# xipengwang/AprilSAM

Hardware: NVIDIA H100
Metric: Gauss-Newton solves/sec (batch + incremental) on M3500 & 100k-pose graph (higher is better)
Workload: dtype f64

## Files before the change

aprilsam_b200/csrc/asam_cuda.cu:

```cuda

#include <cuda_runtime.h>

#include <climits>
#include <cmath>
#include <cstdarg>
#include <cstdint>
#include <cstdio>
#include <cstdlib>
#include <cstring>
#include <ctime>
#include <vector>

#include "asam_cuda.h"

#define ASAM_EXPORT extern "C" __attribute__((visibility("default")))

static thread_local char g_err[512] = "";

static int set_err(const char *fmt, ...)
{
    va_list ap;
    va_start(ap, fmt);
    vsnprintf(g_err, sizeof(g_err), fmt, ap);
    va_end(ap);
// ... 1526 lines not shown
    for (int rep = 0; rep < 4; rep++) {
        CK(cudaEventRecord(d->tev[0], d->stream));
        k_fp64_peak<<<d->n_sm, threads, 0, d->stream>>>((double *) d->partial.p, iters);
        CK(cudaGetLastError());
        CK(cudaEventRecord(d->tev[1], d->stream));
        CK(cudaEventSynchronize(d->tev[1]));
        float ms = 0.f;
        CK(cudaEventElapsedTime(&ms, d->tev[0], d->tev[1]));
        const double tf = 2.0 * 8 * iters * (double) threads * d->n_sm / (ms * 1e-3) * 1e-12;
        if (rep > 0 && tf > best)
            best = tf;
    }
    *tflops_out = best;
    return 0;
}

ASAM_EXPORT int asam_device_info(asam_dev_t *d, int *n_sm, int *fac_grid, int *fac_smem, int *bs_grid)
{
    *n_sm = d->n_sm;
    *fac_grid = d->fac_grid;
    *fac_smem = d->fac_smem;
    *bs_grid = d->bs_grid;
    return 0;
}

ASAM_EXPORT int asam_set_trace(asam_dev_t *d, int enabled)
{
    d->trace_on = enabled;
    return 0;
}

ASAM_EXPORT int asam_download_trace(asam_dev_t *d, int which, unsigned long long *out, int max_tasks)
{
    CK(cudaSetDevice(d->device));
    if (flush_uploads(d))
        return 1;
    int n = which == 0 ? d->trace_nfac : d->trace_nbs;
    Buf &b = which == 0 ? d->trace_fac : d->trace_bs;
    if (n > max_tasks)
        n = max_tasks;
    if (n <= 0 || !b.p)
        return 0;
    CK(cudaMemcpyAsync(out, b.p, (size_t) n * 8 * sizeof(unsigned long long), cudaMemcpyDeviceToHost, d->stream));
    CK(cudaStreamSynchronize(d->stream));
    return 0;
}

ASAM_EXPORT int asam_set_panel_trace(asam_dev_t *d, int sn, int max_panels)
{
    CK(cudaSetDevice(d->device));
    d->ptrace_sn = -1;
    if (sn < 0 || max_panels <= 0)
        return 0;
    const size_t bytes = (size_t) max_panels * 64 * sizeof(unsigned long long);
    if (buf_reserve(d, d->ptrace, bytes, false, false) || flush_uploads(d))
        return 1;
    CK(cudaMemsetAsync(d->ptrace.p, 0, bytes, d->stream));
    d->ptrace_sn = sn;
    d->ptrace_panels = max_panels;
    return 0;
}

ASAM_EXPORT int asam_download_panel_trace(asam_dev_t *d, unsigned long long *out, int max_panels)
{
    CK(cudaSetDevice(d->device));
    if (!d->ptrace.p || max_panels > d->ptrace_panels)
        return set_err("asam_download_panel_trace: no trace");
    if (flush_uploads(d))
        return 1;
    CK(cudaMemcpyAsync(out, d->ptrace.p, (size_t) max_panels * 64 * sizeof(unsigned long long), cudaMemcpyDeviceToHost, d->stream));
    CK(cudaStreamSynchronize(d->stream));
    return 0;
}

ASAM_EXPORT int asam_set_timing(asam_dev_t *d, int enabled)
{
    d->timing = enabled;
    d->ev_set[0] = d->ev_set[1] = d->ev_set[2] = 0;
    return 0;
}

ASAM_EXPORT int asam_last_kernel_ms(asam_dev_t *d, float *lin_ms, float *fac_ms, float *bs_ms)
{
    CK(cudaSetDevice(d->device));
    if (flush_uploads(d))
        return 1;
    CK(cudaStreamSynchronize(d->stream));
    float *outs[3] = { lin_ms, fac_ms, bs_ms };
    for (int i = 0; i < 3; i++) {
        float ms = 0.f;
        if (d->ev_set[i])
            CK(cudaEventElapsedTime(&ms, d->ev[2 * i], d->ev[2 * i + 1]));
        if (outs[i])
            *outs[i] = ms;
    }
    return 0;
}
```

aprilsam_b200/csrc/asam_kernels.cuh:

```cuda
#pragma once

#include <cuda_runtime.h>

#include <cstdint>

#include "asam_cuda.h"

#define ASAM_TR_FLAG (1 << 30)
#define ASAM_MAX_CACHED_CHILDREN 24

__device__ __forceinline__ double d_mod2pi(double v)
{
    const double twopi = 6.2831853071795862319959;
    const double pi = 3.141592653589793238462643383279502884196;
    double w = v + pi;
    return (w - twopi * floor(w / twopi)) - pi;
}

__device__ __forceinline__ void d_atb(const double *A, const double *B, double *C)
{
#pragma unroll
    for (int i = 0; i < 3; i++)
#pragma unroll
        for (int j = 0; j < 3; j++) {
// ... 26 lines not shown
        r[i] = A[i * 3 + 0] * v[0] + A[i * 3 + 1] * v[1] + A[i * 3 + 2] * v[2];
}

__device__ __forceinline__ void d_xyt_eval(const double *pa, const double *pb, const double *z, double *Ja,
                                           double *Jb, double *r)
{
    double ca, sa;
    sincos(pa[2], &sa, &ca);
    double dx = pb[0] - pa[0], dy = pb[1] - pa[1];
    double zh0 = ca * dx + sa * dy;
    double zh1 = -sa * dx + ca * dy;
    double zh2 = pb[2] - pa[2];
    Ja[0] = -ca; Ja[1] = -sa; Ja[2] = -sa * dx + ca * dy;
    Ja[3] = sa;  Ja[4] = -ca; Ja[5] = -ca * dx - sa * dy;
    Ja[6] = 0.0; Ja[7] = 0.0; Ja[8] = -1.0;
    Jb[0] = ca;  Jb[1] = sa;  Jb[2] = 0.0;
    Jb[3] = -sa; Jb[4] = ca;  Jb[5] = 0.0;
    Jb[6] = 0.0; Jb[7] = 0.0; Jb[8] = 1.0;
    r[0] = z[0] - zh0;
    r[1] = z[1] - zh1;
    r[2] = d_mod2pi(z[2] - zh2);
}

__device__ __forceinline__ bool d_two_pose(const int type) { return type == 1 || type == 32; }

__device__ __forceinline__ double d_loss_weight(const int loss, const double k, const double s)
{
    const double k2 = k * k;
    if (loss == 1)
        return s <= k2 ? 1.0 : k / sqrt(s);
    return 1.0 / (1.0 + s / k2);
}

__device__ __forceinline__ double d_loss_rho(const int loss, const double k, const double s)
{
    const double k2 = k * k;
    if (loss == 1)
        return s <= k2 ? s : 2.0 * k * sqrt(s) - k2;
    return k2 * log1p(s / k2);
}

__device__ __forceinline__ double d_rsqrt_in_range(const double a)
{
    double y = (double) rsqrtf((float) a);
    double e = fma(-a * y, y, 1.0);
    y = fma(0.5 * y, e, y);
    e = fma(-a * y, y, 1.0);
    y = fma(0.5 * y, e, y);
    return y;
}

__device__ __forceinline__ double d_rsqrt(const double a)
{
    if (!(a >= 0x1p-120 && a <= 0x1p120)) {
        if (!(a > 0.0 && a < INFINITY))
            return rsqrt(a);
        int ex;
        frexp(a, &ex);
        const int h = ex / 2;
        return ldexp(d_rsqrt_in_range(ldexp(a, -2 * h)), -h);
    }
    return d_rsqrt_in_range(a);
}

__device__ __forceinline__ int ld_volatile(const int *p) { return *((const volatile int *) p); }

__device__ __forceinline__ int ld_acquire(const int *p)
{
    int v;
    asm volatile("ld.acquire.gpu.global.b32 %0, [%1];" : "=r"(v) : "l"(p) : "memory");
    return v;
}
__device__ __forceinline__ void st_release(int *p, const int v)
{
    asm volatile("st.release.gpu.global.b32 [%0], %1;" ::"l"(p), "r"(v) : "memory");
}
__device__ __forceinline__ void red_release_add(int *p, const int v)
{
    asm volatile("red.release.gpu.global.add.s32 [%0], %1;" ::"l"(p), "r"(v) : "memory");
}

__device__ __forceinline__ unsigned long long d_now()
{
    unsigned long long t;
    asm volatile("mov.u64 %0, %%globaltimer;" : "=l"(t));
    return t;
}

struct SpinClock {
    long long n = 0;
    unsigned long long t0 = 0;
};
__device__ __forceinline__ bool spin_over(SpinClock &c, long long limit_ns)
{
    if ((++c.n & 1023) != 0)
        return false;
    const unsigned long long now = d_now();
    if (c.t0 == 0) {
        c.t0 = now;
        return false;
    }
    return (long long) (now - c.t0) > limit_ns;
}


struct LinArgs {
    const int *f_type, *f_a, *f_b, *f_slot;
    const double *f_z, *f_W;
    const double2 *f_loss;
    const double *lp, *st;
    const double *pts;
    const int *node2q;
    double *Adiag, *Aoff, *Bq;
    int f_first, f_count;
};
// ... 299 lines not shown
            const double x2 = (p2[i] - x0 * l20 - x1 * l21) * r2;
            p0[i] = x0;
            p1[i] = x1;
            p2[i] = x2;
        }
        PF_SYNC();
        if (tid == 0) {
            p0[rb] = a00 * r0; p0[rb + 1] = l10; p0[rb + 2] = l20;
            p1[rb + 1] = d1 * r1; p1[rb + 2] = l21;
            p2[rb + 2] = d2 * r2;
            if (dinv_out) {
                dinv_out[rb] = r0; dinv_out[rb + 1] = r1; dinv_out[rb + 2] = r2;
            }
        }
        const int nrem = pb - (c0 + 3);
        const int nrow = m - (rb + 3) + 1;
        if (nrem > 0 && nrow > 0) {
            int ng = g_pf_groups ? nt / nrow : 1;
            ng = ng > nrem ? nrem : ng;
            if (ng > 1) {
                const int gi = tid / nrow, ri = tid - gi * nrow;
                if (gi < ng) {
                    const int i = rb + 3 + ri;
                    const double x0 = p0[i], x1 = p1[i], x2 = p2[i];
                    const int jmax = min(nrem, ri + 1);
                    for (int jj = gi; jj < jmax; jj += ng) {
                        const int jr = rb + 3 + jj;
                        double *pj = P + (size_t) (c0 + 3 + jj) * ldp;
                        pj[i] -= x0 * p0[jr] + x1 * p1[jr] + x2 * p2[jr];
                    }
                }
            } else {
                for (int i = i_first; i <= m; i += nt) {
                    const double x0 = p0[i], x1 = p1[i], x2 = p2[i];
                    const int jmax = min(nrem, i - (rb + 3) + 1);
                    for (int jj = 0; jj < jmax; jj++) {
                        const int jr = rb + 3 + jj;
                        double *pj = P + (size_t) (c0 + 3 + jj) * ldp;
                        pj[i] -= x0 * p0[jr] + x1 * p1[jr] + x2 * p2[jr];
                    }
                }
            }
        }
    }
    PF_SYNC();
#undef PF_SYNC
}

#define ASAM_TPB 48
#define ASAM_TROWS 256
#define ASAM_TCOLS 64

#define ASAM_CROWS 128

__device__ __forceinline__ unsigned smem_u32(const void *p) { return (unsigned) __cvta_generic_to_shared(p); }

__device__ __forceinline__ void mbar_init(unsigned long long *bar, unsigned count)
{
    asm volatile("mbarrier.init.shared::cta.b64 [%0], %1;" ::"r"(smem_u32(bar)), "r"(count) : "memory");
    asm volatile("fence.mbarrier_init.release.cluster;" ::: "memory");
}

__device__ __forceinline__ void mbar_expect_tx(unsigned long long *bar, unsigned bytes)
{
    asm volatile("mbarrier.arrive.expect_tx.shared::cta.b64 _, [%0], %1;" ::"r"(smem_u32(bar)), "r"(bytes) : "memory");
}

__device__ __forceinline__ void mbar_wait(unsigned long long *bar, unsigned parity)
{
    unsigned ok;
    long long tries = 0;
    do {
        asm volatile("{\n\t.reg .pred p;\n\tmbarrier.try_wait.parity.shared::cta.b64 p, [%1], %2;\n\tselp.u32 %0, 1, 0, p;\n\t}"
                     : "=r"(ok)
                     : "r"(smem_u32(bar)), "r"(parity)
                     : "memory");
        if (!ok && ++tries > (1LL << 24))
            __trap();
    } while (!ok);
}

__device__ __forceinline__ void bulk_g2s(void *dst, const void *src, unsigned bytes, unsigned long long *bar)
{
    asm volatile("cp.async.bulk.shared::cluster.global.mbarrier::complete_tx::bytes [%0], [%1], %2, [%3];" ::"r"(smem_u32(dst)),
                 "l"(src), "r"(bytes), "r"(smem_u32(bar))
                 : "memory");
}

#define ASAM_LDW 52
#define ASAM_WS_DOUBLES(m) (2 * (size_t) ((m) + 2) * ASAM_LDW)

template <int MT>
__device__ __noinline__ void tile_rm(double *F, const int ld, const double *Wk, const int pb4, const int cb0, const int ncol,
                                     const int rb0, const int nrow, const int out_mode, double *Out, double *Li, double *Lj,
                                     unsigned long long *bar, unsigned &parity)
{
    const int tid = threadIdx.x;
    const int lane = tid & 31, warp = tid >> 5;
    const bool same = rb0 == cb0 && nrow >= ncol;
    __syncthreads();
    if (warp == 0) {
        asm volatile("fence.proxy.async;" ::: "memory");
        if (lane == 0) {
            const unsigned bi = (unsigned) nrow * ASAM_LDW * 8u, bj = same ? 0u : (unsigned) ncol * ASAM_LDW * 8u;
            mbar_expect_tx(bar, bi + bj);
            bulk_g2s(Li, Wk + (size_t) rb0 * ASAM_LDW, bi, bar);
// ... 56 lines not shown
                        else if (out_mode == 1)
                            Out[ii + jj * ASAM_TPB] = acc[mt][q][e];
                        else
                            Out[ii + jj * ASAM_TROWS] = acc[mt][q][e];
                    }
                }
    }
}

struct TeamCtx {
    int *tbar_s;
    int G, w, phase;
    long long spin_limit;
    int *err;
    int sn;
};

__device__ __forceinline__ bool team_barrier(TeamCtx &tc, int *s_flag)
{
    __syncthreads();
    if (threadIdx.x == 0) {
        red_release_add(tc.tbar_s, 1);
        const int target = (++tc.phase) * tc.G;
        SpinClock spins;
        int ok = 1;
        while (ld_volatile(tc.tbar_s) < target) {
            __nanosleep(20);
            if (spin_over(spins, tc.spin_limit) || ld_volatile(tc.err) < 0) {
                atomicCAS(tc.err, 0, -(1 + tc.sn));
                ok = 0;
                break;
            }
        }
        ld_acquire(tc.tbar_s);
        *s_flag = ok;
    } else {
        tc.phase++;
    }
    __syncthreads();
    return *s_flag != 0;
}

__device__ __forceinline__ void team_leave(TeamCtx &tc)
{
    if (threadIdx.x == 0) {
        const int v = atomicAdd(tc.tbar_s, 1);
        if (v == tc.phase * tc.G + tc.G - 1)
            atomicExch(tc.tbar_s, 0);
    }
}

__device__ __forceinline__ bool team_owns(int col, int w, int G) { return ((col >> 2) % G) == w; }

__device__ __forceinline__ void diag_factor_rl(double *D, int pb, double *rdv, int sn_id, int *err)
{
    constexpr int LDD = ASAM_TPB;
    constexpr int SUB = 256;
    if (threadIdx.x < SUB) {
        for (int k1 = 0; k1 < pb; k1 += ASAM_PB) {
            const int pbb = min(ASAM_PB, pb - k1);
            panel_factor(D + (size_t) k1 * LDD, LDD, k1, pbb, pb - 1, sn_id, err, rdv, SUB);
            if (k1 + pbb < pb) {
                trailing_update_mma(D, LDD, D + (size_t) k1 * LDD, LDD, pbb, k1 + pbb, pb, pb - 1, SUB / 32);
                bar_sub(SUB);
            }
        }
    }
    __syncthreads();
}

__device__ __forceinline__ void trsm_row_block(double *Li, const double *D, const double *rdv, const int b0, const int nb,
                                               double *Frow, int ld, double *Wrow)
{
    const int tid = threadIdx.x;
    constexpr int LDD = ASAM_TPB;
    double r[12];
#pragma unroll
    for (int q = 0; q < 12; q++)
        r[q] = (q < nb) ? Li[tid + (b0 + q) * ASAM_TROWS] : 0.0;
    for (int p = 0; p < b0; p++) {
        const double xp = Li[tid + p * ASAM_TROWS];
        const double2 *Dp = reinterpret_cast<const double2 *>(D + p * LDD + b0);
#pragma unroll
        for (int q2 = 0; q2 < 6; q2++) {
            const double2 v = Dp[q2];
            r[2 * q2] -= xp * v.x;
            r[2 * q2 + 1] -= xp * v.y;
        }
    }
#pragma unroll
    for (int q = 0; q < 12; q++) {
        if (q < nb) {
            r[q] *= rdv[b0 + q];
#pragma unroll
            for (int q2 = q + 1; q2 < 12; q2++)
                r[q2] -= r[q] * D[(b0 + q2) + (b0 + q) * LDD];
        }
    }
#pragma unroll
    for (int q = 0; q < 12; q++)
        if (q < nb) {
            Li[tid + (b0 + q) * ASAM_TROWS] = r[q];
            Frow[(size_t) (b0 + q) * ld] = r[q];
            Wrow[b0 + q] = r[q];
        }
}

__device__ __forceinline__ void trsm_row(double *Li, const double *D, const double *rdv, int pb, double *Frow, int ld,
                                         double *Wrow)
{
    for (int b0 = 0; b0 < pb; b0 += 12)
        trsm_row_block(Li, D, rdv, b0, min(12, pb - b0), Frow, ld, Wrow);
    for (int q = pb; q < ((pb + 3) & ~3); q++)
        Wrow[q] = 0.0;
// ... 106 lines not shown
    if (!team_barrier(tc, s_flag))
        return false;
    if (w == 0 && nw > 0 && tid == 0)
        a.arrive[s] = 0;
    unsigned long long t_panel = 0, t_mark = 0;
    if (trow && tid == 0)
        trow[3] = d_now();

    double *D = sm;
    double *rdv = D + ASAM_TPB * ASAM_TPB;
    double *Li = rdv + ASAM_TPB;
    double *Lj = Li + ASAM_TROWS * ASAM_LDW;
    double *Wbase = F + (size_t) ld * m;
    auto Wbuf = [&](int panel_index) { return Wbase + (size_t) (panel_index & 1) * (m + 2) * ASAM_LDW; };
    double *dinv = a.dinv + 3 * (size_t) d.first;
    int *crew_bar = a.tbar + 2 * (size_t) s + 1;

    auto tile = [&](int k0, int pb, int cb0, int ncol, int rb0, int nrow, double *Dout) {
        const double *Wk = Wbuf(k0 / ASAM_TPB);
        const int pb4 = (pb + 3) & ~3;
        if (Dout)
            tile_rm<1>(F, ld, Wk, pb4, cb0, ncol, rb0, nrow, 1, Dout, Li, Lj, mbar, mb_parity);
        else if (nrow <= 128)
            tile_rm<2>(F, ld, Wk, pb4, cb0, ncol, rb0, nrow, 0, nullptr, Li, Lj, mbar, mb_parity);
        else
            tile_rm<4>(F, ld, Wk, pb4, cb0, ncol, rb0, nrow, 0, nullptr, Li, Lj, mbar, mb_parity);
    };
    auto panel = [&](int k0, int pb, int rb0) {
        __syncthreads();
        for (int e = tid; e < ASAM_TPB * ASAM_TPB; e += nt) {
            const int i = e % ASAM_TPB, j = e / ASAM_TPB;
            D[e] = (i >= j && i < pb && j < pb) ? __ldcg(&F[(k0 + i) + (size_t) (k0 + j) * ld]) : 0.0;
        }
        const int i = rb0 + tid;
        const bool row = rb0 >= 0 && i >= k0 + pb && i <= m;
        if (row)
            for (int j = 0; j < pb; j++)
                Li[tid + j * ASAM_TROWS] = __ldcg(&F[i + (size_t) (k0 + j) * ld]);
        __syncthreads();
        diag_factor_rl(D, pb, rdv, s, err);
        if (row)
            trsm_row(Li, D, rdv, pb, F + i + (size_t) k0 * ld, ld, Wbuf(0) + (size_t) i * ASAM_LDW);
    };
    auto writeback = [&](int k0, int pb) {
        for (int e = tid; e < pb * pb; e += nt) {
            const int i = e % pb, j = e / pb;
            if (i >= j)
                F[(k0 + i) + (size_t) (k0 + j) * ld] = D[i + j * ASAM_TPB];
        }
        for (int e = tid; e < pb; e += nt)
            dinv[k0 + e] = rdv[e];
    };

    auto diag_publish = [&](int k0, int pb, int seq) {
        __syncthreads();
        constexpr int LDD = ASAM_TPB;
        constexpr int SUB = 256;
        int stage = 0;
        for (int k1 = 0; k1 < pb; k1 += ASAM_PB) {
            const int pbb = min(ASAM_PB, pb - k1);
            panel_factor(D + (size_t) k1 * LDD, LDD, k1, pbb, pb - 1, s, err, rdv, SUB);
            ++stage;
            for (int e = tid; e < pbb * pb; e += SUB) {
                const int j = k1 + e / pb, i = e % pb;
                if (i >= j)
                    F[(k0 + i) + (size_t) (k0 + j) * ld] = D[i + j * LDD];
            }
            for (int e = tid; e < pbb; e += SUB)
                dinv[k0 + k1 + e] = rdv[k1 + e];
            bar_sub(SUB);
            if (tid == 0)
                st_release(crew_bar, 8 * seq + stage);
            if (k1 + pbb < pb) {
                trailing_update_mma(D, LDD, D + (size_t) k1 * LDD, LDD, pbb, k1 + pbb, pb, pb - 1, SUB / 32);
                bar_sub(SUB);
            }
        }
        __syncthreads();
    };
    auto rows_solve_staged = [&](int k0, int pb, int rb0, int seq, double *Wnext) {
        constexpr int LDD = ASAM_TPB;
        if (tid == 0)
            *s_flag = 1;
        __syncthreads();
        const int i = rb0 + tid;
        const bool row = tid < ASAM_CROWS && i <= m;
        int stage = 0;
        for (int b0 = 0; b0 < pb; b0 += ASAM_PB, ++stage) {
            const int nb = min(ASAM_PB, pb - b0);
            if (warp >= 4) {
                if (tid == 128 && *s_flag) {
                    SpinClock spins;
                    while (ld_volatile(crew_bar) < 8 * seq + stage + 1) {
                        __nanosleep(20);
                        if (spin_over(spins, a.spin_limit) || ld_volatile(err) < 0) {
                            atomicCAS(err, 0, -(1 + s));
                            *s_flag = 0;
                            break;
                        }
                    }
                    ld_acquire(crew_bar);
                }
                asm volatile("bar.sync 2, 128;" ::: "memory");
                if (*s_flag) {
                    for (int e = tid - 128; e < nb * ASAM_TPB; e += 128) {
                        const int j = b0 + e / ASAM_TPB, ii = e % ASAM_TPB;
                        D[ii + j * LDD] = (ii >= j && ii < pb) ? __ldcg(&F[(k0 + ii) + (size_t) (k0 + j) * ld]) : 0.0;
                    }
                    if (tid - 128 < nb)
                        rdv[b0 + tid - 128] = __ldcg(&dinv[k0 + b0 + tid - 128]);
                }
                __threadfence_block();
                asm volatile("bar.arrive %0, 256;" ::"r"(3 + stage) : "memory");
            } else {
                asm volatile("bar.sync %0, 256;" ::"r"(3 + stage) : "memory");
                if (row && *s_flag)
                    trsm_row_block(Li, D, rdv, b0, nb, F + i + (size_t) k0 * ld, ld, Wnext + (size_t) i * ASAM_LDW);
            }
        }
        if (row && *s_flag)
            for (int q = pb; q < ((pb + 3) & ~3); q++)
                Wnext[(size_t) i * ASAM_LDW + q] = 0.0;
        __syncthreads();
        return *s_flag != 0;
    };
    {
        const int pb = min(ASAM_TPB, c);
        if (trow && tid == 0)
            t_mark = d_now();
        const int nchunk = (m + 1 + ASAM_TROWS - 1) / ASAM_TROWS;
        bool first = true;
        for (int ch = w; ch < nchunk || first; ch += G) {
            panel(0, pb, ch < nchunk ? ch * ASAM_TROWS : -1);
            first = false;
        }
        if (!team_barrier(tc, s_flag))
            return false;
        if (trow && tid == 0)
            t_panel += d_now() - t_mark;
        if (w == 0)
            writeback(0, pb);
    }
    int seq = 0;
    const bool pt_on = a.ptrace && s == a.ptrace_sn && w < 8 && tid == 0;
    for (int k0 = 0; k0 < c; k0 += ASAM_TPB) {
        unsigned long long *pt = (pt_on && k0 / ASAM_TPB < a.ptrace_panels) ? a.ptrace + ((size_t) (k0 / ASAM_TPB) * 8 + w) * 8 : nullptr;
        if (pt) {
            pt[0] = d_now();
            pt[1] = pt[2] = pt[3] = pt[0];
            pt[5] = (unsigned long long) m;
            pt[6] = (unsigned long long) G;
        }
        const int pb = min(ASAM_TPB, c - k0);
        const int kn0 = k0 + pb;
        const bool has_next = kn0 < c;
        const int pbn = has_next ? min(ASAM_TPB, c - kn0) : 0;
        const int ncrew = has_next ? 1 + (m - (kn0 + pbn) + 1 + ASAM_CROWS - 1) / ASAM_CROWS : 0;
        ++seq;
        if (w < ncrew) {
            if (trow && tid == 0)
                t_mark = d_now();
            if (w == 0) {
                __syncthreads();
                for (int e = tid; e < ASAM_TPB * ASAM_TPB; e += nt)
                    D[e] = 0.0;
                tile(k0, pb, kn0, pbn, kn0, pbn, D);
                if (pt)
                    pt[1] = d_now();
                diag_publish(kn0, pbn, seq);
                if (pt)
                    pt[2] = d_now();
            }
            for (int it = (w == 0 ? G : w); it < ncrew; it += G) {
                const int rb0 = kn0 + pbn + (it - 1) * ASAM_CROWS;
                tile_rm<2>(F, ld, Wbuf(k0 / ASAM_TPB), (pb + 3) & ~3, kn0, pbn, rb0, min(ASAM_CROWS, m - rb0 + 1), 2, Li, Li,
                           Lj, mbar, mb_parity);
                if (pt && w > 0 && it == w)
                    pt[1] = d_now();
                if (!rows_solve_staged(kn0, pbn, rb0, seq, Wbuf(kn0 / ASAM_TPB)))
                    return false;
            }
            if (pt && w > 0)
                pt[2] = d_now();
            if (trow && tid == 0)
                t_panel += d_now() - t_mark;
        }

        const int j0 = kn0 + pbn;
        const int nfree = (G - ncrew >= 2) ? G - ncrew : G, wfree = (G - ncrew >= 2) ? w - ncrew : w;
        int n256 = 0;
        for (int cb0 = j0; cb0 < m; cb0 += ASAM_TCOLS)
            n256 += (m - cb0 + 1 + 255) / 256;
        const int TR = (n256 < 2 * nfree) ? 128 : 256;
        if (wfree >= 0) {
            int u = 0;
            for (int cb0 = j0; cb0 < m; cb0 += ASAM_TCOLS)
                for (int rb0 = cb0; rb0 <= m; rb0 += TR, ++u)
                    if (u % nfree == wfree)
                        tile(k0, pb, cb0, min(ASAM_TCOLS, m - cb0), rb0, min(TR, m - rb0 + 1), nullptr);
        }
        if (pt)
            pt[3] = d_now();
        if (!team_barrier(tc, s_flag))
            return false;
        if (pt) {
            pt[4] = d_now();
            pt[7] = (unsigned long long) ncrew;
        }
    }
    if (w == 0 && tid == 0)
        atomicExch(crew_bar, 0);

    if (trow && tid == 0) {
        trow[4] = d_now();
        trow[7] = (unsigned long long) (unsigned) m | (t_panel << 32);
    }
    if (w == 0) {
        for (int e = tid; e < c; e += nt)
            a.y[3 * (size_t) d.first + e] = __ldcg(&F[m + (size_t) e * ld]);
        __syncthreads();
        if (tid == 0 && d.parent >= 0) {
            __threadfence();
            atomicAdd(&a.arrive[d.parent], 1);
        }
    }
    team_leave(tc);
    __syncthreads();
    return true;
}

__device__ __forceinline__ void ticket_release(int *ticket, int *done)
{
// ... 579 lines not shown
            __threadfence();
            atomicAdd(&a.arrive[d.parent], 1);
        }
        __syncwarp();
    }
    ticket_release(&a.ctrl[5], &a.ctrl[6]);
}

struct BsArgs {
    const asam_sn_desc_t *sn;
    const int *ipool;
    const double *arena;
    const double *y;
    const double *dinv;
    double *x;
    int *xdone;
    const int *btasks;
    const int *bfirst;
    int *xblk;
    int ntasks;
    int *ctrl;
    int epoch;
    int smem_doubles;
    long long spin_limit;
    unsigned long long *trace;
};

#define ASAM_BSW 96
#define ASAM_BT_SN(e) ((e) & 0xffffff)
#define ASAM_BT_BLK(e) ((((e) >> 24) & 0x7f) - 1)

template <int U>
__device__ __forceinline__ double bs_dot(const double *lk, const double *xs, int n, int lane)
{
    double acc0 = 0.0, acc1 = 0.0;
    for (int i0 = lane; i0 < n; i0 += 32 * U) {
        double v[U];
#pragma unroll
        for (int u = 0; u < U; u++)
            v[u] = (i0 + 32 * u < n) ? lk[i0 + 32 * u] : 0.0;
#pragma unroll
        for (int u = 0; u < U; u += 2) {
            acc0 += v[u] * xs[min(i0 + 32 * u, n - 1)];
            acc1 += v[u + 1] * xs[min(i0 + 32 * (u + 1), n - 1)];
        }
    }
    acc0 += acc1;
#pragma unroll
    for (int o = 16; o > 0; o >>= 1)
        acc0 += __shfl_down_sync(0xffffffffu, acc0, o);
    return acc0;
}

__device__ bool cta_backsolve(const BsArgs &a, const int t, const int s, double *sm, int *s_abort, const int jcol = 0,
                              const int blk_only = -1)
{
    const int tid = threadIdx.x, nt = blockDim.x;
    const int lane = tid & 31, warp = tid >> 5, nwarps = nt >> 5;
    int *err = a.ctrl + 1;
    unsigned long long tr0 = 0, tr1 = 0, tr2 = 0;
    if (a.trace && tid == 0)
        tr0 = d_now();
    const asam_sn_desc_t d = a.sn[s];
    const int m = 3 * d.mb, c = 3 * d.cb, r = m - c, ld = ASAM_LD(m);
    const int *rows = a.ipool + d.seg;
    const double *Lg = a.arena + d.f_off;
    const int bwmax = min(c, ASAM_BSW);
    if (m + 2 * bwmax + 2 > a.smem_doubles) {
        if (tid == 0)
            atomicCAS(err, 0, -(1 + s));
        return false;
    }
    double *xf = sm;
    double *w = sm + m;
    double *rd = w + bwmax;
    double *Ls = rd + bwmax;
    const long long room = (long long) a.smem_doubles - (m + 2 * bwmax);
    const int nblk = (c + ASAM_BSW - 1) / ASAM_BSW;

    const int blk_hi = blk_only >= 0 ? blk_only : nblk - 1, blk_lo = blk_only >= 0 ? blk_only : 0;
    for (int blk = blk_hi; blk >= blk_lo; --blk) {
        const int b0 = blk * ASAM_BSW, bw = min(ASAM_BSW, c - b0), be = b0 + bw, hb = m - b0;
        if (be <= jcol)
            break;
        const int kmin = max(0, jcol - b0);
        const int lm = hb | 1, lc = bw | 1;
        const int mode = ((long long) lm * bw <= room) ? 2 : (((long long) lc * bw <= room) ? 1 : 0);
        const int ll = mode == 2 ? lm : (mode == 1 ? lc : ld);
        if (blk != blk_hi)
            __syncthreads();
        if (mode == 2) {
            for (int k = kmin + warp; k < bw; k += nwarps)
                for (int i = k + lane; i < hb; i += 32)
                    Ls[i + (size_t) k * lm] = Lg[(b0 + i) + (size_t) (b0 + k) * ld];
        } else if (mode == 1) {
            for (int k = kmin + warp; k < bw; k += nwarps)
                for (int i = k + lane; i < bw; i += 32)
                    Ls[i + (size_t) k * lc] = Lg[(b0 + i) + (size_t) (b0 + k) * ld];
        }
        for (int k = tid; k < bw; k += nt) {
            w[k] = a.y[3 * (size_t) d.first + b0 + k];
            rd[k] = a.dinv[3 * (size_t) d.first + b0 + k];
        }
        const double *L11 = mode ? Ls : (Lg + b0 + (size_t) b0 * ld);

        if (blk == blk_hi) {
            if (a.trace && tid == 0)
                tr1 = d_now();
            if (d.parent >= 0 && tid == 0) {
                SpinClock spins;
                while (ld_volatile(&a.xdone[d.parent]) != a.epoch) {
                    __nanosleep(20);
                    if (spin_over(spins, a.spin_limit) || ld_volatile(err) < 0) {
                        atomicCAS(err, 0, -(1 + s));
                        *s_abort = 1;
                        break;
                    }
                }
                __threadfence();
            }
            __syncthreads();
            if (*s_abort)
                break;
            if (a.trace && tid == 0)
                tr2 = d_now();
            for (int i = tid; i < r; i += nt)
                xf[c + i] = __ldcg(&a.x[3 * (size_t) rows[d.cb + i / 3] + i % 3]);
        }
        __syncthreads();
        if (blk_only >= 0) {
            if (r > 0) {
                for (int k = warp; k < bw; k += nwarps) {
                    const double *lk = (mode == 2) ? (Ls + (size_t) k * lm + (c - b0)) : (Lg + (size_t) (b0 + k) * ld + c);
                    const double acc = r > 512 ? bs_dot<16>(lk, xf + c, r, lane) : bs_dot<8>(lk, xf + c, r, lane);
                    if (lane == 0)
                        w[k] -= acc;
                }
            }
            const int ep = a.epoch & 0xffffff;
            for (int b2 = nblk - 1; b2 > blk; --b2) {
                const int r0 = b2 * ASAM_BSW, n2 = min(ASAM_BSW, c - r0), need = nblk - b2;
                if (tid == 0) {
                    SpinClock spins;
                    for (;;) {
                        const int v = ld_volatile(&a.xblk[s]);
                        if ((int) ((unsigned) v >> 8) == ep && (v & 0xff) >= need)
                            break;
                        __nanosleep(20);
                        if (spin_over(spins, a.spin_limit) || ld_volatile(err) < 0) {
                            atomicCAS(err, 0, -(1 + s));
                            *s_abort = 1;
                            break;
                        }
                    }
                    __threadfence();
                }
                __syncthreads();
                if (*s_abort)
                    break;
                for (int i = tid; i < n2; i += nt)
                    xf[r0 + i] = __ldcg(&a.x[3 * (size_t) d.first + r0 + i]);
                __syncthreads();
                {
                    double xv[3];
#pragma unroll
                    for (int u = 0; u < 3; u++)
                        xv[u] = lane + 32 * u < n2 ? xf[r0 + lane + 32 * u] : 0.0;
#pragma unroll 1
                    for (int j0 = 0; j0 * nwarps < bw; j0 += 6) {
                        double lv[6][3];
#pragma unroll
                        for (int j = 0; j < 6; j++) {
                            const int k = warp + nwarps * (j0 + j);
                            const double *lk = (mode == 2) ? (Ls + (size_t) min(k, bw - 1) * lm + (r0 - b0))
                                                           : (Lg + (size_t) (b0 + min(k, bw - 1)) * ld + r0);
#pragma unroll
                            for (int u = 0; u < 3; u++)
                                lv[j][u] = (k < bw && lane + 32 * u < n2) ? lk[lane + 32 * u] : 0.0;
                        }
#pragma unroll
                        for (int j = 0; j < 6; j++) {
                            double acc = lv[j][0] * xv[0] + lv[j][1] * xv[1] + lv[j][2] * xv[2];
#pragma unroll
                            for (int o = 16; o > 0; o >>= 1)
                                acc += __shfl_down_sync(0xffffffffu, acc, o);
                            const int k = warp + nwarps * (j0 + j);
                            if (lane == 0 && k < bw)
                                w[k] -= acc;
                        }
                    }
                }
            }
            __syncthreads();
            if (*s_abort)
                break;
        }
        const int nr = blk_only >= 0 ? 0 : m - be;
        if (nr > 0) {
            for (int k = kmin + warp; k < bw; k += nwarps) {
                const double *lk = (mode == 2) ? (Ls + (size_t) k * lm + bw) : (Lg + (size_t) (b0 + k) * ld + be);
                const double acc = nr > 512 ? bs_dot<16>(lk, xf + be, nr, lane) : bs_dot<8>(lk, xf + be, nr, lane);
                if (lane == 0)
                    w[k] -= acc;
            }
            __syncthreads();
        }
        if (warp == 0) {
            double wr[3];
#pragma unroll
            for (int t3 = 0; t3 < 3; t3++)
                wr[t3] = (lane + 32 * t3 < bw) ? w[lane + 32 * t3] : 0.0;
#pragma unroll 2
            for (int k = bw - 1; k >= kmin; --k) {
                const int ks = k >> 5;
                const double mine = ks == 0 ? wr[0] : (ks == 1 ? wr[1] : wr[2]);
                const double xk = __shfl_sync(0xffffffffu, mine, k & 31) * rd[k];
#pragma unroll
                for (int t3 = 0; t3 < 3; t3++) {
                    const int j = lane + 32 * t3;
                    if (j < k && j >= kmin)
                        wr[t3] -= L11[k + (size_t) j * ll] * xk;
                    else if (j == k)
                        wr[t3] = xk;
                }
            }
#pragma unroll
            for (int t3 = 0; t3 < 3; t3++) {
                const int k = lane + 32 * t3;
                if (k < bw && k >= kmin) {
                    a.x[3 * (size_t) d.first + b0 + k] = wr[t3];
                    xf[b0 + k] = wr[t3];
                }
            }
            __syncwarp();
        }
    }
    if (*s_abort)
        return false;
    if (warp == 0 && lane == 0) {
        __threadfence();
        if (blk_only >= 0)
            atomicExch(&a.xblk[s], ((a.epoch & 0xffffff) << 8) | (nblk - blk_only));
        if (blk_only <= 0)
            atomicExch(&a.xdone[s], a.epoch);
        if (a.trace) {
            unsigned long long *tr = a.trace + 8 * (size_t) t;
            tr[0] = tr0; tr[1] = tr1; tr[2] = tr2; tr[3] = d_now();
            tr[6] = (unsigned long long) s;
            tr[7] = (unsigned) m;
        }
    }
    __syncthreads();
    return true;
}

__global__ void __launch_bounds__(256, 2) k_backsolve(BsArgs a)
{
    extern __shared__ __align__(16) double sm[];
    __shared__ int s_task, s_abort;
    const int tid = threadIdx.x, nt = blockDim.x;
    const int lane = tid & 31, warp = tid >> 5, nwarps = nt >> 5;
    int *err = a.ctrl + 1;

    for (;;) {
        if (tid == 0) {
            s_task = atomicAdd(&a.ctrl[2], 1);
            s_abort = 0;
        }
        __syncthreads();
        const int t = s_task;
        if (t >= a.ntasks)
            break;
        if (!cta_backsolve(a, t, ASAM_BT_SN(a.btasks[t]), sm, &s_abort, a.bfirst ? 3 * a.bfirst[t] : 0, ASAM_BT_BLK(a.btasks[t])))
            break;
    }
    ticket_release(&a.ctrl[2], &a.ctrl[4]);
}

#define ASAM_BSL_WARPS 8
#define ASAM_BSL_PANEL 1024
#define ASAM_BSL_XS 64
#define ASAM_BSL_STRIDE (ASAM_BSL_PANEL + ASAM_BSL_XS)

__global__ void __launch_bounds__(32 * ASAM_BSL_WARPS) k_backsolve_leaf(BsArgs a)
{
    extern __shared__ __align__(16) double sm[];
    const int lane = threadIdx.x & 31, warp = threadIdx.x >> 5;
    double *Ls = sm + (size_t) warp * ASAM_BSL_STRIDE;
    double *xs = Ls + ASAM_BSL_PANEL;
    int *err = a.ctrl + 1;
    for (;;) {
        int t = 0;
        if (lane == 0)
            t = atomicAdd(&a.ctrl[5], 1);
        t = __shfl_sync(0xffffffffu, t, 0);
        if (t >= a.ntasks)
            break;
        const int s = ASAM_BT_SN(a.btasks[t]);
        const asam_sn_desc_t d = a.sn[s];
        const int m = 3 * d.mb, c = 3 * d.cb, r = m - c, ld = ASAM_LD(m);
        if (r > ASAM_BSL_XS || c > 64) {
            if (lane == 0)
                atomicCAS(err, 0, -(1 + s));
            break;
        }
        const int *rows = a.ipool + d.seg;
        const double *Lg = a.arena + d.f_off;
        const int lm = m | 1;
        const bool staged = lm * c <= ASAM_BSL_PANEL;
        if (staged) {
            for (int k = 0; k < c; k++)
                for (int i = k + lane; i < m; i += 32)
                    Ls[i + k * lm] = Lg[i + (size_t) k * ld];
        }
        const double *L = staged ? Ls : Lg;
        const int ll = staged ? lm : ld;
        double wr[2], rdv[2];
#pragma unroll
        for (int t2 = 0; t2 < 2; t2++) {
            const int k = lane + 32 * t2;
            wr[t2] = k < c ? a.y[3 * (size_t) d.first + k] : 0.0;
            rdv[t2] = k < c ? a.dinv[3 * (size_t) d.first + k] : 0.0;
        }
        int abort_ = 0;
        if (d.parent >= 0) {
            if (lane == 0) {
                SpinClock spins;
                while (ld_volatile(&a.xdone[d.parent]) != a.epoch) {
                    __nanosleep(20);
                    if (spin_over(spins, a.spin_limit) || ld_volatile(err) < 0) {
                        atomicCAS(err, 0, -(1 + s));
                        abort_ = 1;
                        break;
                    }
                }
                __threadfence();
            }
            abort_ = __shfl_sync(0xffffffffu, abort_, 0);
        }
        if (abort_)
            break;
        for (int i = lane; i < r; i += 32)
            xs[i] = __ldcg(&a.x[3 * (size_t) rows[d.cb + i / 3] + i % 3]);
        __syncwarp();
#pragma unroll
        for (int t2 = 0; t2 < 2; t2++) {
            const int k = lane + 32 * t2;
            if (k < c) {
                const double *lk = L + c + (size_t) k * ll;
                double acc0 = 0.0, acc1 = 0.0;
                int i = 0;
#pragma unroll 4
                for (; i + 1 < r; i += 2) {
                    acc0 += lk[i] * xs[i];
                    acc1 += lk[i + 1] * xs[i + 1];
                }
                if (i < r)
                    acc0 += lk[i] * xs[i];
                wr[t2] -= acc0 + acc1;
            }
        }
        for (int k = c - 1; k >= 0; --k) {
            const double mine = (k >> 5) == 0 ? wr[0] : wr[1];
            const double rk = (k >> 5) == 0 ? rdv[0] : rdv[1];
            const double xk = __shfl_sync(0xffffffffu, mine * rk, k & 31);
#pragma unroll
            for (int t2 = 0; t2 < 2; t2++) {
                const int j = lane + 32 * t2;
                if (j < k)
                    wr[t2] -= L[k + (size_t) j * ll] * xk;
                else if (j == k)
                    wr[t2] = xk;
            }
        }
#pragma unroll
        for (int t2 = 0; t2 < 2; t2++) {
            const int k = lane + 32 * t2;
            if (k < c)
                a.x[3 * (size_t) d.first + k] = wr[t2];
        }
        __syncwarp();
        if (lane == 0) {
            __threadfence();
            atomicExch(&a.xdone[s], a.epoch);
        }
        __syncwarp();
    }
    ticket_release(&a.ctrl[5], &a.ctrl[6]);
}

struct StepArgs {
    const uint4 *host_in;
    uint4 *stage;
    unsigned int table_bytes, payload_off, payload_bytes;
    int n_items;
    LinArgs lin;
    FacArgs fac;
    BsArgs bs;
    double *x_out;
    volatile int *done;
    int seq;
};

__global__ void __launch_bounds__(256, 1) k_step(StepArgs a)
{
    extern __shared__ __align__(16) double sm[];
    __shared__ int s_abort;
    __shared__ asam_sn_desc_t s_cd[ASAM_MAX_CACHED_CHILDREN];
    const int tid = threadIdx.x, nt = blockDim.x, lane = tid & 31, warp = tid >> 5, nwarps = nt >> 5;
    volatile unsigned long long *stamps = (volatile unsigned long long *) (a.done + 2);
    if (tid == 0)
        stamps[0] = d_now();

    {
        const unsigned nt16 = (a.table_bytes + 15) >> 4, np16 = (a.payload_bytes + 15) >> 4, p0 = a.payload_off >> 4;
        const unsigned n16 = nt16 + np16;
        for (unsigned i0 = tid; i0 < n16; i0 += 4 * nt) {
            uint4 v[4];
#pragma unroll
            for (int u = 0; u < 4; u++) {
                const unsigned i = i0 + u * nt;
                if (i < n16)
                    v[u] = a.host_in[i < nt16 ? i : p0 + (i - nt16)];
            }
#pragma unroll
            for (int u = 0; u < 4; u++) {
                const unsigned i = i0 + u * nt;
                if (i < n16)
                    a.stage[i < nt16 ? i : p0 + (i - nt16)] = v[u];
            }
        }
    }
    __syncthreads();
    {
        const BatchItem *items = (const BatchItem *) a.stage;
        const char *payload = (const char *) a.stage + a.payload_off;
        for (int it = warp; it < a.n_items; it += nwarps) {
            const BatchItem bi = items[it];
// ... 389 lines not shown
```

Measured before the change: 143.6.

## Overlap diagonal publish with trailing update and use specialized 3-column subpanel factor

Replaces the generic panel_factor in the diagonal-block Cholesky with a specialized diag_subpanel that factors three columns at a time in registers and defers writes. In diag_publish, a dedicated 64-thread group writes the factored subpanel and dinv back to global memory and releases the crew barrier, while the other 192 threads run the trailing MMA update concurrently. This shortens the critical path that the row-solve crews wait on. It also reorders d_rsqrt to compute the fast path first, and widens the panel trace to record per-stage timestamps. The trailing update now runs with fewer warps.

Result: faster. 147.9 (median of 6 runs) (+3.0%).

```diff
diff --git a/aprilsam_b200/csrc/asam_cuda.cu b/aprilsam_b200/csrc/asam_cuda.cu
--- a/aprilsam_b200/csrc/asam_cuda.cu
+++ b/aprilsam_b200/csrc/asam_cuda.cu
@@ -1602,7 +1602,7 @@
     d->ptrace_sn = -1;
     if (sn < 0 || max_panels <= 0)
         return 0;
-    const size_t bytes = (size_t) max_panels * 64 * sizeof(unsigned long long);
+    const size_t bytes = (size_t) max_panels * 8 * ASAM_PT_WORDS * sizeof(unsigned long long);
     if (buf_reserve(d, d->ptrace, bytes, false, false) || flush_uploads(d))
         return 1;
     CK(cudaMemsetAsync(d->ptrace.p, 0, bytes, d->stream));
@@ -1618,7 +1618,7 @@
         return set_err("asam_download_panel_trace: no trace");
     if (flush_uploads(d))
         return 1;
-    CK(cudaMemcpyAsync(out, d->ptrace.p, (size_t) max_panels * 64 * sizeof(unsigned long long), cudaMemcpyDeviceToHost, d->stream));
+    CK(cudaMemcpyAsync(out, d->ptrace.p, (size_t) max_panels * 8 * ASAM_PT_WORDS * sizeof(unsigned long long), cudaMemcpyDeviceToHost, d->stream));
     CK(cudaStreamSynchronize(d->stream));
     return 0;
 }
diff --git a/aprilsam_b200/csrc/asam_kernels.cuh b/aprilsam_b200/csrc/asam_kernels.cuh
--- a/aprilsam_b200/csrc/asam_kernels.cuh
+++ b/aprilsam_b200/csrc/asam_kernels.cuh
@@ -102,15 +102,15 @@
 
 __device__ __forceinline__ double d_rsqrt(const double a)
 {
-    if (!(a >= 0x1p-120 && a <= 0x1p120)) {
-        if (!(a > 0.0 && a < INFINITY))
-            return rsqrt(a);
-        int ex;
-        frexp(a, &ex);
-        const int h = ex / 2;
-        return ldexp(d_rsqrt_in_range(ldexp(a, -2 * h)), -h);
-    }
-    return d_rsqrt_in_range(a);
+    const double y = d_rsqrt_in_range(a);
+    if (a >= 0x1p-120 && a <= 0x1p120)
+        return y;
+    if (!(a > 0.0 && a < INFINITY))
+        return rsqrt(a);
+    int ex;
+    frexp(a, &ex);
+    const int h = ex / 2;
+    return ldexp(d_rsqrt_in_range(ldexp(a, -2 * h)), -h);
 }
 
 __device__ __forceinline__ int ld_volatile(const int *p) { return *((const volatile int *) p); }
@@ -516,6 +516,8 @@
 #define ASAM_TCOLS 64
 
 #define ASAM_CROWS 128
+#define ASAM_PT_WORDS 32
+#define ASAM_PT_STAGE 8
 
 __device__ __forceinline__ unsigned smem_u32(const void *p) { return (unsigned) __cvta_generic_to_shared(p); }
 
@@ -678,6 +680,73 @@
 
 __device__ __forceinline__ bool team_owns(int col, int w, int G) { return ((col >> 2) % G) == w; }
 
+__device__ __forceinline__ void diag_subpanel(double *P, const int k0, const int pb, const int m, const int sn_id, int *err,
+                                              double *rdv)
+{
+    constexpr int LDD = ASAM_TPB;
+    const int tid = threadIdx.x, gi = tid >> 6, ri = tid & 63;
+    double *wrow = nullptr, *wdiag = nullptr;
+    double w0 = 0.0, w1 = 0.0, w2 = 0.0, v00 = 0.0, v10 = 0.0, v20 = 0.0, v11 = 0.0, v21 = 0.0, v22 = 0.0;
+    auto flush = [&]() {
+        if (wrow) {
+            wrow[0] = w0; wrow[LDD] = w1; wrow[2 * LDD] = w2;
+            wrow = nullptr;
+        }
+        if (wdiag) {
+            wdiag[0] = v00; wdiag[1] = v10; wdiag[2] = v20;
+            wdiag[LDD + 1] = v11; wdiag[LDD + 2] = v21;
+            wdiag[2 * LDD + 2] = v22;
+            wdiag = nullptr;
+        }
+    };
+    for (int c0 = 0; c0 < pb; c0 += 3) {
+        const int rb = k0 + c0;
+        double *p0 = P + (size_t) c0 * LDD, *p1 = p0 + LDD, *p2 = p1 + LDD;
+        bar_sub(256);
+        const double a00 = p0[rb], a10 = p0[rb + 1], a20 = p0[rb + 2];
+        const double a11 = p1[rb + 1], a21 = p1[rb + 2], a22 = p2[rb + 2];
+        flush();
+        const double r0 = d_rsqrt(a00);
+        const double l10 = a10 * r0, l20 = a20 * r0;
+        const double d1 = a11 - l10 * l10;
+        const double r1 = d_rsqrt(d1);
+        const double l21 = (a21 - l20 * l10) * r1;
+        const double d2 = a22 - l20 * l20 - l21 * l21;
+        const double r2 = d_rsqrt(d2);
+        if (tid == 0) {
+            if (!(a00 > 0.0 && d1 > 0.0 && d2 > 0.0))
+                atomicCAS(err, 0, 1 + sn_id);
+            rdv[rb] = r0; rdv[rb + 1] = r1; rdv[rb + 2] = r2;
+            wdiag = p0 + rb;
+            v00 = a00 * r0; v10 = l10; v20 = l20;
+            v11 = d1 * r1; v21 = l21;
+            v22 = d2 * r2;
+        }
+        const int nrow = m - (rb + 3) + 1, nrem = pb - (c0 + 3);
+        if (ri < nrow && (gi == 0 || gi < nrem)) {
+            const int i = rb + 3 + ri;
+            const double x0 = p0[i] * r0;
+            const double x1 = (p1[i] - x0 * l10) * r1;
+            const double x2 = (p2[i] - x0 * l20 - x1 * l21) * r2;
+            if (gi == 0) {
+                wrow = p0 + i;
+                w0 = x0; w1 = x1; w2 = x2;
+            }
+            const int ng = min(4, nrem), jmax = min(nrem, ri + 1);
+            for (int jj = gi; jj < jmax; jj += ng) {
+                const int jr = rb + 3 + jj;
+                const double y0 = p0[jr] * r0;
+                const double y1 = (p1[jr] - y0 * l10) * r1;
+                const double y2 = (p2[jr] - y0 * l20 - y1 * l21) * r2;
+                double *pj = P + (size_t) (c0 + 3 + jj) * LDD;
+                pj[i] -= x0 * y0 + x1 * y1 + x2 * y2;
+            }
+        }
+    }
+    flush();
+    bar_sub(256);
+}
+
 __device__ __forceinline__ void diag_factor_rl(double *D, int pb, double *rdv, int sn_id, int *err)
 {
     constexpr int LDD = ASAM_TPB;
@@ -685,7 +754,7 @@
     if (threadIdx.x < SUB) {
         for (int k1 = 0; k1 < pb; k1 += ASAM_PB) {
             const int pbb = min(ASAM_PB, pb - k1);
-            panel_factor(D + (size_t) k1 * LDD, LDD, k1, pbb, pb - 1, sn_id, err, rdv, SUB);
+            diag_subpanel(D + (size_t) k1 * LDD, k1, pbb, pb - 1, sn_id, err, rdv);
             if (k1 + pbb < pb) {
                 trailing_update_mma(D, LDD, D + (size_t) k1 * LDD, LDD, pbb, k1 + pbb, pb, pb - 1, SUB / 32);
                 bar_sub(SUB);
@@ -898,33 +967,42 @@
             dinv[k0 + e] = rdv[e];
     };
 
-    auto diag_publish = [&](int k0, int pb, int seq) {
+    auto diag_publish = [&](int k0, int pb, int seq, unsigned long long *ptw) {
         __syncthreads();
         constexpr int LDD = ASAM_TPB;
         constexpr int SUB = 256;
+        constexpr int PUB0 = 192;
+        unsigned long long *pt = tid == 0 ? ptw : nullptr, *ptp = tid == PUB0 ? ptw : nullptr;
         int stage = 0;
         for (int k1 = 0; k1 < pb; k1 += ASAM_PB) {
             const int pbb = min(ASAM_PB, pb - k1);
-            panel_factor(D + (size_t) k1 * LDD, LDD, k1, pbb, pb - 1, s, err, rdv, SUB);
+            diag_subpanel(D + (size_t) k1 * LDD, k1, pbb, pb - 1, s, err, rdv);
+            if (pt)
+                pt[ASAM_PT_STAGE + 4 * stage] = d_now();
+            if (tid >= PUB0) {
+                const int i = tid - PUB0;
+                if (i < pb)
+                    for (int j = k1; j < k1 + pbb && j <= i; j++)
+                        F[(k0 + i) + (size_t) (k0 + j) * ld] = D[i + j * LDD];
+                if (i < pbb)
+                    dinv[k0 + k1 + i] = rdv[k1 + i];
+                if (ptp)
+                    ptp[ASAM_PT_STAGE + 4 * stage + 1] = d_now();
+                asm volatile("bar.sync 7, 64;" ::: "memory");
+                if (tid == PUB0)
+                    st_release(crew_bar, 8 * seq + stage + 1);
+                if (ptp)
+                    ptp[ASAM_PT_STAGE + 4 * stage + 2] = d_now();
+            } else if (k1 + pbb < pb) {
+                trailing_update_mma(D, LDD, D + (size_t) k1 * LDD, LDD, pbb, k1 + pbb, pb, pb - 1, PUB0 / 32);
+            }
+            if (pt)
+                pt[ASAM_PT_STAGE + 4 * stage + 3] = d_now();
             ++stage;
-            for (int e = tid; e < pbb * pb; e += SUB) {
-                const int j = k1 + e / pb, i = e % pb;
-                if (i >= j)
-                    F[(k0 + i) + (size_t) (k0 + j) * ld] = D[i + j * LDD];
-            }
-            for (int e = tid; e < pbb; e += SUB)
-                dinv[k0 + k1 + e] = rdv[k1 + e];
-            bar_sub(SUB);
-            if (tid == 0)
-                st_release(crew_bar, 8 * seq + stage);
-            if (k1 + pbb < pb) {
-                trailing_update_mma(D, LDD, D + (size_t) k1 * LDD, LDD, pbb, k1 + pbb, pb, pb - 1, SUB / 32);
-                bar_sub(SUB);
-            }
         }
         __syncthreads();
     };
-    auto rows_solve_staged = [&](int k0, int pb, int rb0, int seq, double *Wnext) {
+    auto rows_solve_staged = [&](int k0, int pb, int rb0, int seq, double *Wnext, unsigned long long *ptw) {
         constexpr int LDD = ASAM_TPB;
         if (tid == 0)
             *s_flag = 1;
@@ -946,6 +1024,8 @@
                         }
                     }
                     ld_acquire(crew_bar);
+                    if (ptw && stage < 4)
+                        ptw[ASAM_PT_STAGE + stage] = d_now();
                 }
                 asm volatile("bar.sync 2, 128;" ::: "memory");
                 if (*s_flag) {
@@ -962,6 +1042,8 @@
                 asm volatile("bar.sync %0, 256;" ::"r"(3 + stage) : "memory");
                 if (row && *s_flag)
                     trsm_row_block(Li, D, rdv, b0, nb, F + i + (size_t) k0 * ld, ld, Wnext + (size_t) i * ASAM_LDW);
+                if (ptw && tid == 0 && stage < 4)
+                    ptw[ASAM_PT_STAGE + 4 + stage] = d_now();
             }
         }
         if (row && *s_flag)
@@ -988,9 +1070,11 @@
             writeback(0, pb);
     }
     int seq = 0;
-    const bool pt_on = a.ptrace && s == a.ptrace_sn && w < 8 && tid == 0;
+    const bool pt_on = a.ptrace && s == a.ptrace_sn && w < 8;
     for (int k0 = 0; k0 < c; k0 += ASAM_TPB) {
-        unsigned long long *pt = (pt_on && k0 / ASAM_TPB < a.ptrace_panels) ? a.ptrace + ((size_t) (k0 / ASAM_TPB) * 8 + w) * 8 : nullptr;
+        unsigned long long *ptw =
+            (pt_on && k0 / ASAM_TPB < a.ptrace_panels) ? a.ptrace + ((size_t) (k0 / ASAM_TPB) * 8 + w) * ASAM_PT_WORDS : nullptr;
+        unsigned long long *pt = tid == 0 ? ptw : nullptr;
         if (pt) {
             pt[0] = d_now();
             pt[1] = pt[2] = pt[3] = pt[0];
@@ -1013,7 +1097,7 @@
                 tile(k0, pb, kn0, pbn, kn0, pbn, D);
                 if (pt)
                     pt[1] = d_now();
-                diag_publish(kn0, pbn, seq);
+                diag_publish(kn0, pbn, seq, ptw);
                 if (pt)
                     pt[2] = d_now();
             }
@@ -1023,7 +1107,7 @@
                            Lj, mbar, mb_parity);
                 if (pt && w > 0 && it == w)
                     pt[1] = d_now();
-                if (!rows_solve_staged(kn0, pbn, rb0, seq, Wbuf(kn0 / ASAM_TPB)))
+                if (!rows_solve_staged(kn0, pbn, rb0, seq, Wbuf(kn0 / ASAM_TPB), it == w ? ptw : nullptr))
                     return false;
             }
             if (pt && w > 0)
```

## Block backsolve triangular steps by 3 and use acquire/release flags

Applied to the files above, without the earlier changes.

Rewrites the warp-level triangular back-substitution in both the CTA and warp backsolve paths to process three columns per step. A small 3x3 solve is done redundantly per lane, which cuts the serial shuffle chain by a factor of three. Replaces threadfence plus atomicExch signalling with ld_acquire/st_release. In the blocked path, L loads for the first twelve rows are prefetched into registers before spinning on the dependency flag, so they overlap with the wait. This adds register pressure and relies on block widths being multiples of 3; it also extends the trace fields.

New measurement: 143.6 before, 145.2 after (median of 6 runs). 1.01x the previous value.

```diff
diff --git a/aprilsam_b200/csrc/asam_kernels.cuh b/aprilsam_b200/csrc/asam_kernels.cuh
--- a/aprilsam_b200/csrc/asam_kernels.cuh
+++ b/aprilsam_b200/csrc/asam_kernels.cuh
@@ -1709,15 +1709,50 @@
     return acc0;
 }
 
+__device__ __forceinline__ void bs_warp_solve(const double *L11, const int ll, const double *rd, double (&wr)[3],
+                                              const int bw, const int kmin, const int lane)
+{
+    const double *col[3];
+#pragma unroll
+    for (int t3 = 0; t3 < 3; t3++)
+        col[t3] = L11 + (size_t) min(lane + 32 * t3, bw - 1) * ll;
+#pragma unroll 2
+    for (int k = bw - 3; k >= kmin; k -= 3) {
+        double wk[3];
+#pragma unroll
+        for (int q = 0; q < 3; q++) {
+            const int ks = (k + q) >> 5;
+            wk[q] = __shfl_sync(0xffffffffu, ks == 0 ? wr[0] : (ks == 1 ? wr[1] : wr[2]), (k + q) & 31);
+        }
+        const double *pk = L11 + (size_t) k * ll + k;
+        const double x2 = wk[2] * rd[k + 2];
+        wk[1] -= pk[2 + ll] * x2;
+        wk[0] -= pk[2] * x2;
+        const double x1 = wk[1] * rd[k + 1];
+        wk[0] -= pk[1] * x1;
+        const double x0 = wk[0] * rd[k];
+#pragma unroll
+        for (int t3 = 0; t3 < 3; t3++) {
+            const int j = lane + 32 * t3;
+            const double *cj = col[t3] + k;
+            double v = wr[t3];
+            v -= cj[2] * x2;
+            v -= cj[1] * x1;
+            v -= cj[0] * x0;
+            wr[t3] = (j < k && j >= kmin) ? v : (j == k ? x0 : (j == k + 1 ? x1 : (j == k + 2 ? x2 : wr[t3])));
+        }
+    }
+}
+
 __device__ bool cta_backsolve(const BsArgs &a, const int t, const int s, double *sm, int *s_abort, const int jcol = 0,
                               const int blk_only = -1)
 {
     const int tid = threadIdx.x, nt = blockDim.x;
     const int lane = tid & 31, warp = tid >> 5, nwarps = nt >> 5;
     int *err = a.ctrl + 1;
-    unsigned long long tr0 = 0, tr1 = 0, tr2 = 0;
-    if (a.trace && tid == 0)
-        tr0 = d_now();
+    unsigned long long *tr = a.trace ? a.trace + 8 * (size_t) t : nullptr;
+    if (tr && tid == 0)
+        tr[0] = d_now();
     const asam_sn_desc_t d = a.sn[s];
     const int m = 3 * d.mb, c = 3 * d.cb, r = m - c, ld = ASAM_LD(m);
     const int *rows = a.ipool + d.seg;
@@ -1759,11 +1794,10 @@
             w[k] = a.y[3 * (size_t) d.first + b0 + k];
             rd[k] = a.dinv[3 * (size_t) d.first + b0 + k];
         }
-        const double *L11 = mode ? Ls : (Lg + b0 + (size_t) b0 * ld);
 
         if (blk == blk_hi) {
-            if (a.trace && tid == 0)
-                tr1 = d_now();
+            if (tr && tid == 0)
+                tr[1] = d_now();
             if (d.parent >= 0 && tid == 0) {
                 SpinClock spins;
                 while (ld_volatile(&a.xdone[d.parent]) != a.epoch) {
@@ -1774,17 +1808,19 @@
                         break;
                     }
                 }
-                __threadfence();
+                ld_acquire(&a.xdone[d.parent]);
             }
             __syncthreads();
             if (*s_abort)
                 break;
-            if (a.trace && tid == 0)
-                tr2 = d_now();
+            if (tr && tid == 0)
+                tr[4] = tr[2] = d_now();
             for (int i = tid; i < r; i += nt)
                 xf[c + i] = __ldcg(&a.x[3 * (size_t) rows[d.cb + i / 3] + i % 3]);
         }
         __syncthreads();
+        if (tr && tid == 0 && blk == blk_hi)
+            tr[5] = d_now();
         if (blk_only >= 0) {
             if (r > 0) {
                 for (int k = warp; k < bw; k += nwarps) {
@@ -1797,6 +1833,16 @@
             const int ep = a.epoch & 0xffffff;
             for (int b2 = nblk - 1; b2 > blk; --b2) {
                 const int r0 = b2 * ASAM_BSW, n2 = min(ASAM_BSW, c - r0), need = nblk - b2;
+                double lv[12][3];
+#pragma unroll
+                for (int j = 0; j < 12; j++) {
+                    const int k = warp + nwarps * j;
+                    const double *lk = (mode == 2) ? (Ls + (size_t) min(k, bw - 1) * lm + (r0 - b0))
+                                                   : (Lg + (size_t) (b0 + min(k, bw - 1)) * ld + r0);
+#pragma unroll
+                    for (int u = 0; u < 3; u++)
+                        lv[j][u] = (k < bw && lane + 32 * u < n2) ? lk[lane + 32 * u] : 0.0;
+                }
                 if (tid == 0) {
                     SpinClock spins;
                     for (;;) {
@@ -1810,21 +1856,35 @@
                             break;
                         }
                     }
-                    __threadfence();
+                    ld_acquire(&a.xblk[s]);
                 }
                 __syncthreads();
                 if (*s_abort)
                     break;
+                if (tr && tid == 0)
+                    tr[4] = d_now();
                 for (int i = tid; i < n2; i += nt)
                     xf[r0 + i] = __ldcg(&a.x[3 * (size_t) d.first + r0 + i]);
                 __syncthreads();
+                if (tr && tid == 0)
+                    tr[5] = d_now();
                 {
                     double xv[3];
 #pragma unroll
                     for (int u = 0; u < 3; u++)
                         xv[u] = lane + 32 * u < n2 ? xf[r0 + lane + 32 * u] : 0.0;
+#pragma unroll
+                    for (int j = 0; j < 12; j++) {
+                        double acc = lv[j][0] * xv[0] + lv[j][1] * xv[1] + lv[j][2] * xv[2];
+#pragma unroll
+                        for (int o = 16; o > 0; o >>= 1)
+                            acc += __shfl_down_sync(0xffffffffu, acc, o);
+                        const int k = warp + nwarps * j;
+                        if (lane == 0 && k < bw)
+                            w[k] -= acc;
+                    }
 #pragma unroll 1
-                    for (int j0 = 0; j0 * nwarps < bw; j0 += 6) {
+                    for (int j0 = 12; j0 * nwarps < bw; j0 += 6) {
                         double lv[6][3];
 #pragma unroll
                         for (int j = 0; j < 6; j++) {
@@ -1862,25 +1922,17 @@
             }
             __syncthreads();
         }
+        if (tr && tid == 0 && blk == blk_hi)
+            tr[5] = ((tr[5] - tr[4]) << 32) | (d_now() - tr[4]);
         if (warp == 0) {
             double wr[3];
 #pragma unroll
             for (int t3 = 0; t3 < 3; t3++)
                 wr[t3] = (lane + 32 * t3 < bw) ? w[lane + 32 * t3] : 0.0;
-#pragma unroll 2
-            for (int k = bw - 1; k >= kmin; --k) {
-                const int ks = k >> 5;
-                const double mine = ks == 0 ? wr[0] : (ks == 1 ? wr[1] : wr[2]);
-                const double xk = __shfl_sync(0xffffffffu, mine, k & 31) * rd[k];
-#pragma unroll
-                for (int t3 = 0; t3 < 3; t3++) {
-                    const int j = lane + 32 * t3;
-                    if (j < k && j >= kmin)
-                        wr[t3] -= L11[k + (size_t) j * ll] * xk;
-                    else if (j == k)
-                        wr[t3] = xk;
-                }
-            }
+            if (mode)
+                bs_warp_solve(Ls, ll, rd, wr, bw, kmin, lane);
+            else
+                bs_warp_solve(Lg + b0 + (size_t) b0 * ld, ld, rd, wr, bw, kmin, lane);
 #pragma unroll
             for (int t3 = 0; t3 < 3; t3++) {
                 const int k = lane + 32 * t3;
@@ -1895,14 +1947,12 @@
     if (*s_abort)
         return false;
     if (warp == 0 && lane == 0) {
-        __threadfence();
         if (blk_only >= 0)
-            atomicExch(&a.xblk[s], ((a.epoch & 0xffffff) << 8) | (nblk - blk_only));
+            st_release(&a.xblk[s], ((a.epoch & 0xffffff) << 8) | (nblk - blk_only));
         if (blk_only <= 0)
-            atomicExch(&a.xdone[s], a.epoch);
-        if (a.trace) {
-            unsigned long long *tr = a.trace + 8 * (size_t) t;
-            tr[0] = tr0; tr[1] = tr1; tr[2] = tr2; tr[3] = d_now();
+            st_release(&a.xdone[s], a.epoch);
+        if (tr) {
+            tr[3] = d_now();
             tr[6] = (unsigned long long) s;
             tr[7] = (unsigned) m;
         }
@@ -1991,8 +2041,9 @@
                         break;
                     }
                 }
-                __threadfence();
-            }
+                ld_acquire(&a.xdone[d.parent]);
+            }
+            __syncwarp();
             abort_ = __shfl_sync(0xffffffffu, abort_, 0);
         }
         if (abort_)
@@ -2017,17 +2068,28 @@
                 wr[t2] -= acc0 + acc1;
             }
         }
-        for (int k = c - 1; k >= 0; --k) {
-            const double mine = (k >> 5) == 0 ? wr[0] : wr[1];
-            const double rk = (k >> 5) == 0 ? rdv[0] : rdv[1];
-            const double xk = __shfl_sync(0xffffffffu, mine * rk, k & 31);
+        for (int k = c - 3; k >= 0; k -= 3) {
+            double wk[3], rk[3];
+#pragma unroll
+            for (int q = 0; q < 3; q++) {
+                const int hi = (k + q) >> 5;
+                wk[q] = __shfl_sync(0xffffffffu, hi == 0 ? wr[0] : wr[1], (k + q) & 31);
+                rk[q] = __shfl_sync(0xffffffffu, hi == 0 ? rdv[0] : rdv[1], (k + q) & 31);
+            }
+            const double x2 = wk[2] * rk[2];
+            wk[1] -= L[(k + 2) + (size_t) (k + 1) * ll] * x2;
+            wk[0] -= L[(k + 2) + (size_t) k * ll] * x2;
+            const double x1 = wk[1] * rk[1];
+            wk[0] -= L[(k + 1) + (size_t) k * ll] * x1;
+            const double x0 = wk[0] * rk[0];
 #pragma unroll
             for (int t2 = 0; t2 < 2; t2++) {
                 const int j = lane + 32 * t2;
-                if (j < k)
-                    wr[t2] -= L[k + (size_t) j * ll] * xk;
-                else if (j == k)
-                    wr[t2] = xk;
+                double v = wr[t2];
+                v -= L[(k + 2) + (size_t) min(j, c - 1) * ll] * x2;
+                v -= L[(k + 1) + (size_t) min(j, c - 1) * ll] * x1;
+                v -= L[k + (size_t) min(j, c - 1) * ll] * x0;
+                wr[t2] = j < k ? v : (j == k ? x0 : (j == k + 1 ? x1 : (j == k + 2 ? x2 : wr[t2])));
             }
         }
 #pragma unroll
@@ -2037,10 +2099,8 @@
                 a.x[3 * (size_t) d.first + k] = wr[t2];
         }
         __syncwarp();
-        if (lane == 0) {
-            __threadfence();
-            atomicExch(&a.xdone[s], a.epoch);
-        }
+        if (lane == 0)
+            st_release(&a.xdone[s], a.epoch);
         __syncwarp();
     }
     ticket_release(&a.ctrl[5], &a.ctrl[6]);
```
